# yangao07/abPOA

Hardware: NVIDIA H100
Metric: GCUPS (DP cells/s), global/convex 10 kbp (higher is better)
Workload: dtype int16 (packed int16x2 DPX arithmetic; int32 kernel only as overflow fallback)

## Files before the change

abpoa_b200/csrc/poa_chain.cu:

```cuda
#include <cuda_runtime.h>
#include <algorithm>
#include <atomic>
#include <chrono>
#include <mutex>
#include <thread>
#include <vector>
#include <stddef.h>
#include <stdio.h>
#include <stdlib.h>
#include <string.h>
#include <unistd.h>
#include "abpoa_gpu.h"
#include "poa_internal.h"
#include "poa_engine.h"
#include "poa_device.cuh"
#include "poa_chain.cuh"
#include "poa_chain_host.h"

#define CK(call) do { cudaError_t e_ = (call); if (e_ != cudaSuccess) \
    poa_die("libabpoa_b200/chain", "%s failed at %s:%d: %s", #call, __FILE__, __LINE__, cudaGetErrorString(e_)); } while (0)

extern "C" cudaError_t poa_launch_chain_dp_worker(int gap_mode, const int *gaps, PoaChainSlot *slots, PoaChainSync *sync, int n_groups,
                                                  const PoaChainParams *cp, int strand, int ps, int ext, const PoaParamsDev *prm, int ring_rows,
                                                  int ring_cells, cudaStream_t st);
extern "C" cudaError_t poa_launch_chain_align_p16(int gap_mode, const int *gaps, const PoaChainSlot *slots, const int32_t *idx, int n_jobs, int round,
                                                  const PoaChainParams *cp, int strand, int ps, int ext, const PoaParamsDev *prm, int ring_rows,
                                                  int ring_cells, cudaStream_t st);
extern "C" void poa_pick_ring(int gap_mode, int bits, int band_cells, size_t smem_budget, int *ring_rows, int *ring_cells);

static_assert(offsetof(PoaChainSync, q_tail) == 128 && offsetof(PoaChainSync, total) == 256 && offsetof(PoaChainSync, abort) == 384,
              "every polled / bumped word of PoaChainSync sits in its own 128-byte line");
static_assert(POA_GFA_HDR_WORDS == POA_GFA_HDR, "the device's GFA record header is the one poa_gfa_from_record reads");

template <bool PS, bool LG>
__global__ void __launch_bounds__(POA_CHAIN_T) poa_chain_seed_kernel(PoaChainSlot *slots, const PoaChainParams *cp, int n) {
    if ((int)blockIdx.x >= n) return;
    chain_seed<PS, LG>(&slots[blockIdx.x], cp);
}

template <bool PS, bool LG, bool KO = false>
__global__ void __launch_bounds__(POA_CHAIN_T) poa_chain_fuse_kernel(PoaChainSlot *slots, const int32_t *idx, const PoaChainParams *cp, int n, int round) {
    if ((int)blockIdx.x >= n) return;
    chain_fuse<PS, LG, KO>(&slots[idx[blockIdx.x]], cp, round);
}

__device__ __forceinline__ int sync_ld(const int32_t *p) { int v; asm volatile("ld.relaxed.gpu.global.s32 %0, [%1];" : "=r"(v) : "l"(p) : "memory"); return v; }
__device__ __forceinline__ void sync_st(int32_t *p, int v) { asm volatile("st.relaxed.gpu.global.s32 [%0], %1;" :: "l"(p), "r"(v) : "memory"); }
__device__ __forceinline__ unsigned long long sync_now_ns() { unsigned long long t; asm volatile("mov.u64 %0, %%globaltimer;" : "=l"(t)); return t; }

template <bool PS, bool LG, bool KO = false>
__global__ void __launch_bounds__(POA_CHAIN_T) poa_chain_fuse_worker_kernel(PoaChainSlot *slots, PoaChainSync *sync, const PoaChainParams *cp) {
    __shared__ int task_s;
    for (;;) {
        if (threadIdx.x < 32) {
            unsigned ticket = 0;
            if (threadIdx.x == 0) ticket = atomicAdd(&sync->q_head, 1u);
            ticket = __shfl_sync(0xffffffffu, ticket, 0);
            int g = -2; unsigned ns = 250, polls = 0;
            const unsigned long long t0 = sync_now_ns(), limit = sync->watchdog_ns;
            const int32_t *tasks = sync->tasks;
            for (;;) {
                if ((polls++ & 31u) == 0) {
                    const int tot = __shfl_sync(0xffffffffu, sync_ld(&sync->total), 0), ab = __shfl_sync(0xffffffffu, sync_ld(&sync->abort), 0);
                    if ((long long)ticket >= (long long)tot || ab) { g = -2; break; }
                    const unsigned late = __shfl_sync(0xffffffffu, (unsigned)(polls > 1 && sync_now_ns() - t0 > limit), 0);
                    if (late) { if (threadIdx.x == 0) sync_st(&sync->abort, 1); g = -2; break; }
                }
                g = __shfl_sync(0xffffffffu, sync_ld(&tasks[ticket]), 0);
                if (g >= 0) break;
                __nanosleep(ns); if (ns < 4000) ns <<= 1;
            }
            if (threadIdx.x == 0) task_s = g;
        }
        __syncthreads();
        const int g = task_s;
        __syncthreads();
        if (g < 0) return;
        __threadfence();
        PoaChainSlot *s = &slots[g];
        const unsigned long long t0 = sync_now_ns();
        chain_fuse<PS, LG, KO>(s, cp, 0);
        __syncthreads();
        __threadfence();
        __syncthreads();
// ... 746 lines not shown
            int khz = 0; if (cudaDeviceGetAttribute(&khz, cudaDevAttrClockRate, c.dev) != cudaSuccess || khz <= 0) khz = 1965000;
            for (int t = 0; t < nw; ++t) {
                dp_ms += (double)(fin[t].fwd_clk + fin[t].bt_clk) / (double)khz; fuse_ms += (double)fin[t].fuse_ns * 1e-6; wait_ms += (double)fin[t].wait_ns * 1e-6;
                n_marks += fin[t].fused > 0 ? fin[t].fused - 1 : 0;
            }
        } else {
            for (Cohort &k : coh)
                for (size_t j = 0; j + 2 < k.marks.size(); j += 3) {
                    float a = 0.f, b = 0.f;
                    CK(cudaEventElapsedTime(&a, k.marks[j], k.marks[j + 1])); CK(cudaEventElapsedTime(&b, k.marks[j + 1], k.marks[j + 2]));
                    dp_ms += a; fuse_ms += b; ++n_marks;
                }
        }
        if (PoaChainStats *stats = c.stats) {
            stats->device_ms += dev_ms; stats->cells += cells; stats->alignments += alns; stats->launches += launches;
            stats->h2d_bytes += h2d; stats->d2h_bytes += d2h; stats->groups_done += nw - n_failed; stats->groups_failed += n_failed;
            stats->fwd_clk += fwd_clk; stats->bt_clk += bt_clk;
            stats->dp_ms += dp_ms; stats->fuse_ms += fuse_ms; stats->dp_launches += n_marks; stats->fuse_launches += n_marks;
            stats->wait_ms += wait_ms; stats->free_running = c.free_run ? 1 : 0;
        }
        if (!c.verbose) return;
#ifdef POA_KPROF
        {
            double pf[6] = {0, 0, 0, 0, 0, 0}; double na = 0;
            for (int t = 0; t < nw; ++t) { for (int z = 0; z < 6; ++z) pf[z] += (double)fin[t].prof[z]; na += fin[t].fused > 0 ? fin[t].fused - 1 : 0; }
            double bd[5] = {0, 0, 0, 0, 0};
            for (int t = 0; t < nw; ++t) for (int z = 0; z < 5; ++z) bd[z] += (double)fin[t].btdiag[z];
            if (na > 0) fprintf(stderr, "[chain, backtrace per alignment] %.0f steps in %.0f speculative rounds, %.0f general steps costing %.0f k-cycles, "
                                        "%.1f rows with their F planes recomputed\n", bd[0] / na, bd[1] / na, bd[2] / na, bd[3] / na, bd[4] / na);
            if (na > 0) fprintf(stderr, "[chain, k-cycles/alignment] -DPOA_KPROF phases: setup %.0f pred %.0f compute %.0f store %.0f rowmax %.0f tail+prefetch %.0f\n",
                                pf[0] / na / 1e3, pf[1] / na / 1e3, pf[2] / na / 1e3, pf[3] / na / 1e3, pf[4] / na / 1e3, pf[5] / na / 1e3);
        }
#endif
        if (c.free_run)
            fprintf(stderr, "[chain] free-running: per group on average %.1f ms inside alignments + %.1f ms inside fuse (waited %.1f ms for fuse workers incl. the fuse itself), %lld alignments\n",
                    dp_ms / nw, fuse_ms / nw, wait_ms / nw, (long long)n_marks);
        else
            fprintf(stderr, "[chain] DP kernels %.1f ms + fuse kernels %.1f ms summed over %zu concurrent cohort streams (%lld rounds)\n", dp_ms, fuse_ms, coh.size(), (long long)n_marks);
        fprintf(stderr, "[chain] wave of %d groups (%zu cohorts, K=%d): stage %.0f + upload-enqueue %.0f + launch-enqueue %.0f ms, stage+launch+device %.0f ms (device %.1f ms), export copy %.0f ms, import+consensus %.0f ms; "
                        "static %.2f GB, pool %.2f GB, export %.1f MB; %d groups handed to the launch engine\n",
                nw, coh.size(), c.K, t_staged - t_wave0, t_uploaded - t_staged, t_enqueued - t_uploaded, t_dev_done - t_wave0, dev_ms, t_copied - t_dev_done, now_ms() - t_copied,
                (double)doff / 1e9, (double)pool_bytes / 1e9, (double)tot_words * 4 / 1e6, n_failed);
    }
};

}

int poa_chain_run(int dev, poa_arena *arena, abpoa_para_t *abpt, int n_workers, const abpoa_gpu_group_t *groups,
                  abpoa_gpu_group_result_t *results, const std::vector<int> &todo, int flags, std::vector<int> &fallback, PoaChainStats *stats,
                  struct PoaEmit *emit) {
    CK(cudaSetDevice(dev));
    const ChainCall c = chain_call(dev, arena, abpt, n_workers, groups, results, todo, flags, stats, emit);
    const std::vector<GroupPlan> plans = plan_groups(c, todo, fallback);
    if (plans.empty()) return 0;
    for (const std::pair<size_t, size_t> &w : split_waves(plans, poa_arena_capacity(arena), fallback))
        Wave(c, plans.data() + w.first, (int)(w.second - w.first), fallback).run();
    return 0;
}
```

abpoa_b200/csrc/poa_chain.cuh:

```cuda
#ifndef POA_CHAIN_CUH
#define POA_CHAIN_CUH

#include <math.h>
#include <stdint.h>
#include "poa_device.cuh"

#ifdef POA_CHAIN_EMUL
#define POA_DEV static inline
#define POA_PAR_FOR(i, n) for (int i = 0; i < (n); ++i)
#define POA_CTA_SYNC() do { } while (0)
#define POA_TID0 1
#define POA_SHARED static
#define POA_ATOMIC_OR(p, v) (*(p) |= (v))
#define POA_CTZ64(x) __builtin_ctzll(x)
#define POA_CHAIN_T 256
#else
#define POA_DEV __device__ __forceinline__
#define POA_PAR_FOR(i, n) for (int i = (int)threadIdx.x; i < (n); i += (int)blockDim.x)
#define POA_CTA_SYNC() __syncthreads()
#define POA_TID0 (threadIdx.x == 0)
#define POA_SHARED __shared__
#define POA_ATOMIC_OR(p, v) atomicOr((p), (v))
#define POA_CTZ64(x) (__ffsll((long long)(x)) - 1)
#define POA_CHAIN_T 256
#endif

#define POA_CF_NODE_CAP   0x01
#define POA_CF_EDGE_CAP   0x02
#define POA_CF_ALN_CAP    0x04
#define POA_CF_ORDER      0x08
#define POA_CF_BLOB_CAP   0x10
#define POA_CF_DP_STATUS  0x20
#define POA_CF_CIGAR      0x40
#define POA_CF_POOL       0x80

#define POA_ST_SKIP       9

typedef struct PoaChainParams {
    int32_t K, A;
    int32_t m, max_mat, min_mis, o1, e1, oe1, oe2;
    int32_t record;
    int32_t P;
    int32_t W;
    int32_t cons_algrm;
    int32_t amb_strand;
} PoaChainParams;

typedef struct PoaChainSlot {
    int32_t n_nodes, n_cap, pred_cap, blob_cap;
    int32_t failed;
    int32_t n_reads, fused;
    int32_t retry;
    int32_t cur;
    int64_t cells;
    int64_t fwd_clk, bt_clk;
    uint8_t *base;
    int32_t *in_cnt, *out_cnt, *aln_cnt, *n_read;
    int32_t *in_id, *in_w, *out_id, *out_w;
    int32_t *aln_id;
    int32_t *order[2];
    int32_t *node_row;
    int32_t *rem_row;
    int32_t *scr[6];
    const uint8_t *reads; const int32_t *read_off;
    const int32_t *read_w;
    PoaJobDesc jd;
    uint8_t *pool_base; unsigned long long *pool_cursor; uint64_t pool_units;
    int32_t turn;
    int32_t rsv0;
    unsigned long long wait_ns, fuse_ns;
    int64_t prof[6];
    int64_t btdiag[5];
    int32_t *rec_score, *rec_nops; uint64_t *rec_hash;
    uint64_t *read_set;
    uint8_t *read_rc;
    uint64_t *rc_cigar;
    PoaResultDev *rc_result;
    const uint8_t *read_qw;
} PoaChainSlot;

template <class Take>
static inline void chain_slot_layout(PoaChainSlot *s, int n_cap, int qmax, int n_reads, int K, int A, int m, int W, bool record, Take take,
                                     bool strand = false, bool ps = false) {
    const size_t nc = (size_t)n_cap, scr_n = nc > (size_t)qmax + 2 ? nc : (size_t)qmax + 2;
    s->n_cap = n_cap; s->pred_cap = (int32_t)(nc * 3); s->n_reads = n_reads;
    s->blob_cap = (int32_t)(256 + (nc + 1) * 8 + (size_t)s->pred_cap * 4 + 4 + (size_t)qmax + 64);
    if (ps) s->blob_cap += (int32_t)((size_t)s->pred_cap * 4 + 4 + 16);
    s->jd.cigar_cap = (int32_t)(qmax + n_cap + 8);
    s->base = (uint8_t *)take(nc);
    s->in_cnt = (int32_t *)take(nc * 4); s->out_cnt = (int32_t *)take(nc * 4); s->aln_cnt = (int32_t *)take(nc * 4); s->n_read = (int32_t *)take(nc * 4);
    s->in_id = (int32_t *)take(nc * K * 4); s->in_w = (int32_t *)take(nc * K * 4); s->out_id = (int32_t *)take(nc * K * 4); s->out_w = (int32_t *)take(nc * K * 4);
    s->aln_id = (int32_t *)take(nc * A * 4);
    s->order[0] = (int32_t *)take(nc * 4); s->order[1] = (int32_t *)take(nc * 4); s->node_row = (int32_t *)take(nc * 4); s->rem_row = (int32_t *)take(nc * 4);
    for (int k = 0; k < 6; ++k) s->scr[k] = (int32_t *)take(scr_n * 4);
    s->jd.blob = (uint8_t *)take((size_t)s->blob_cap);
    s->jd.rowinfo = (PoaRowInfo *)take(nc * sizeof(PoaRowInfo)); s->jd.rowoff = (PoaRowOff *)take(nc * sizeof(PoaRowOff));
    s->jd.cigar = (uint64_t *)take((size_t)s->jd.cigar_cap * 8);
    s->jd.qprof = (int16_t *)take((size_t)m * ((((size_t)qmax + 1 + 7) & ~(size_t)7) + 8) * 2);
    s->jd.result = (PoaResultDev *)take(sizeof(PoaResultDev));
    s->jd.btrec = (PoaBtRec *)take(nc * sizeof(PoaBtRec));
    if (record) { s->rec_score = (int32_t *)take((size_t)n_reads * 4); s->rec_nops = (int32_t *)take((size_t)n_reads * 4); s->rec_hash = (uint64_t *)take((size_t)n_reads * 8); }
    if (W > 0) s->read_set = (uint64_t *)take(nc * W * 8);
    if (strand) {
        s->read_rc = (uint8_t *)take((size_t)n_reads);
        s->rc_cigar = (uint64_t *)take((size_t)s->jd.cigar_cap * 8);
        s->rc_result = (PoaResultDev *)take(sizeof(PoaResultDev));
    }
}

template <class Take>
static inline void chain_slot_reads(PoaChainSlot *s, int n_reads, int64_t bases, Take take, bool qv = false) {
    s->reads = (const uint8_t *)take((size_t)bases);
    s->read_off = (const int32_t *)take(((size_t)n_reads + 1) * 4);
    s->read_w = (const int32_t *)take((size_t)n_reads * 4);
    if (qv) s->read_qw = (const uint8_t *)take((size_t)bases);
}

typedef struct PoaChainSync {
    unsigned int q_head; int32_t pad0[31];
    unsigned int q_tail; int32_t pad1[31];
    int32_t total; int32_t pad2[31];
    int32_t abort; int32_t pad3[31];
    unsigned long long watchdog_ns;
    int32_t *tasks;
} PoaChainSync;

#ifdef POA_CHAIN_EMUL
POA_DEV int cta_excl_scan(int32_t *a, int n) {
    int run = 0;
    for (int i = 0; i < n; ++i) { const int v = a[i]; a[i] = run; run += v; }
    return run;
}
POA_DEV void cta_incl_maxscan(int32_t *a, int n) {
    int run = INT32_MIN;
    for (int i = 0; i < n; ++i) { if (a[i] > run) run = a[i]; a[i] = run; }
}
#else
__device__ inline int cta_excl_scan(int32_t *a, int n) {
    __shared__ int warp_sum[32];
    __shared__ int carry_s;
    const int lane = threadIdx.x & 31, wid = threadIdx.x >> 5, nw = blockDim.x >> 5;
    if (threadIdx.x == 0) carry_s = 0;
    __syncthreads();
    for (int base = 0; base < n; base += blockDim.x) {
        const int i = base + threadIdx.x;
        const int v = i < n ? a[i] : 0;
        int x = v;
#pragma unroll
        for (int d = 1; d < 32; d <<= 1) { const int t = __shfl_up_sync(0xffffffffu, x, d); if (lane >= d) x += t; }
        if (lane == 31) warp_sum[wid] = x;
        __syncthreads();
        if (wid == 0) {
            int s = lane < nw ? warp_sum[lane] : 0;
#pragma unroll
            for (int d = 1; d < 32; d <<= 1) { const int t = __shfl_up_sync(0xffffffffu, s, d); if (lane >= d) s += t; }
            warp_sum[lane] = s;
        }
        __syncthreads();
        const int carry = carry_s;
        const int before = carry + (wid > 0 ? warp_sum[wid - 1] : 0) + x - v;
        if (i < n) a[i] = before;
        __syncthreads();
        if (threadIdx.x == 0) carry_s = carry + warp_sum[nw - 1];
        __syncthreads();
    }
    return carry_s;
}
__device__ inline void cta_incl_maxscan(int32_t *a, int n) {
    __shared__ int warp_max[32];
    __shared__ int carry_m;
    const int lane = threadIdx.x & 31, wid = threadIdx.x >> 5, nw = blockDim.x >> 5;
    if (threadIdx.x == 0) carry_m = INT32_MIN;
    __syncthreads();
    for (int base = 0; base < n; base += blockDim.x) {
        const int i = base + threadIdx.x;
        int x = i < n ? a[i] : INT32_MIN;
#pragma unroll
        for (int d = 1; d < 32; d <<= 1) { const int t = __shfl_up_sync(0xffffffffu, x, d); if (lane >= d) x = max(x, t); }
        if (lane == 31) warp_max[wid] = x;
        __syncthreads();
        if (wid == 0) {
            int s = lane < nw ? warp_max[lane] : INT32_MIN;
#pragma unroll
            for (int d = 1; d < 32; d <<= 1) { const int t = __shfl_up_sync(0xffffffffu, s, d); if (lane >= d) s = max(s, t); }
            warp_max[lane] = s;
        }
        __syncthreads();
        int r = max(carry_m, x);
        if (wid > 0) r = max(r, warp_max[wid - 1]);
        if (i < n) a[i] = r;
        __syncthreads();
        if (threadIdx.x == 0) carry_m = max(carry_m, warp_max[nw - 1]);
        __syncthreads();
    }
}
#endif

POA_DEV void chain_exchange_order(int32_t *ids, int32_t *ws, int n) {
    for (int j = 0; j + 1 < n; ++j)
        for (int k = j + 1; k < n; ++k)
            if (ws[j] < ws[k]) { int32_t t = ids[j]; ids[j] = ids[k]; ids[k] = t; t = ws[j]; ws[j] = ws[k]; ws[k] = t; }
}

POA_DEV int chain_group_last_row(const PoaChainSlot *s, int A, const int32_t *order, int old_n, int v) {
    int r = s->node_row[v];
    const int na = s->aln_cnt[v];
    if (na == 0) return r;
    const int32_t *al = s->aln_id + (size_t)v * A;
    for (; r + 1 < old_n; ++r) {
        const int u = order[r + 1];
        int member = 0;
        for (int a = 0; a < na; ++a) if (al[a] == u) { member = 1; break; }
        if (!member) break;
    }
    return r;
}

POA_DEV int chain_ref_pn(const PoaChainParams *cp, int qlen, int n_rows) {
    const int len = qlen > n_rows ? qlen : n_rows;
    const int a = qlen * cp->max_mat, b = len * cp->e1 + cp->o1;
    const int max_score = a > b ? a : b;
    return max_score <= 32767 - cp->min_mis - cp->oe1 - cp->oe2 ? 16 : 8;
}

#define POA_LG_ROW_CELLS(pn) (2 * ((pn) - 1))

POA_DEV size_t chain_al16(size_t x) { return (x + 15) & ~(size_t)15; }

POA_DEV bool chain_weak_hit(int best_score, int qlen, int node_n, int max_mat) {
    const int lim = qlen < node_n - 2 ? qlen : node_n - 2;
    return best_score < lim * max_mat * .3333;
}

#define POA_PS_MAX_NODE_W (1 << 20)
POA_DEV int chain_path_score(int edge_w, int node_w) {
    if (node_w == 0 || edge_w == 0) return 0;
    const int s = (int)round(log((double)edge_w / (double)node_w));
    return s > -20 ? s : -20;
}

POA_DEV uint8_t chain_comp(uint8_t b) { return b < 4 ? (uint8_t)(3 - b) : (uint8_t)4; }

typedef struct ChainRead { const uint8_t *q, *w; int len; bool rc; } ChainRead;

POA_DEV ChainRead chain_read(const PoaChainSlot *s, int r) {
    ChainRead rd;
    rd.q = s->reads + s->read_off[r]; rd.w = s->read_qw ? s->read_qw + s->read_off[r] : NULL;
    rd.len = s->read_off[r + 1] - s->read_off[r]; rd.rc = s->read_rc && (s->read_rc[r] & 1);
    return rd;
}

POA_DEV uint8_t chain_read_base(const ChainRead &rd, int qi) { return rd.rc ? chain_comp(rd.q[rd.len - 1 - qi]) : rd.q[qi]; }

POA_DEV int chain_read_weight(const ChainRead &rd, int qi) { return !rd.w ? 1 : rd.w[rd.rc ? rd.len - 1 - qi : qi]; }

POA_DEV void chain_set_remain(PoaChainSlot *s, int K, const int32_t *order, int n) {
    POA_SHARED int t_ptr[POA_CHAIN_T], t_val[POA_CHAIN_T], t_np[POA_CHAIN_T], t_nv[POA_CHAIN_T];
    int32_t *rem = s->rem_row;
    if (POA_TID0) rem[n - 1] = -1;
    POA_CTA_SYNC();
    for (int hi = n - 1; hi > 0; hi -= POA_CHAIN_T) {
        const int lo = hi - POA_CHAIN_T > 0 ? hi - POA_CHAIN_T : 0;
        const int cnt = hi - lo;
        POA_PAR_FOR(l, POA_CHAIN_T) {
            if (l < cnt) {
                const int v = order[lo + l];
                const int sr = s->node_row[s->out_id[(size_t)v * K]];
                if (sr >= hi) { t_ptr[l] = -1; t_val[l] = rem[sr] + 1; }
                else { t_ptr[l] = sr - lo; t_val[l] = 1; }
            } else { t_ptr[l] = -1; t_val[l] = 0; }
        }
        POA_CTA_SYNC();
        for (int step = 1; step < POA_CHAIN_T; step <<= 1) {
            POA_PAR_FOR(l, POA_CHAIN_T) {
                const int p = t_ptr[l];
                if (p >= 0) { t_nv[l] = t_val[l] + t_val[p]; t_np[l] = t_ptr[p]; } else { t_nv[l] = t_val[l]; t_np[l] = -1; }
            }
            POA_CTA_SYNC();
            POA_PAR_FOR(l, POA_CHAIN_T) { t_val[l] = t_nv[l]; t_ptr[l] = t_np[l]; }
            POA_CTA_SYNC();
        }
        POA_PAR_FOR(l, POA_CHAIN_T) { if (l < cnt) rem[lo + l] = t_val[l]; }
        POA_CTA_SYNC();
    }
}

#define CHAIN_KAHN_LINK 0xff
POA_DEV void chain_kahn_order(PoaChainSlot *s, const PoaChainParams *cp, int32_t *order, int n) {
    const int K = cp->K, A = cp->A;
    uint8_t *deg = reinterpret_cast<uint8_t *>(s->scr[2]);
    int32_t *nx = s->scr[3];
    POA_PAR_FOR(v, n) {
        const int ni = s->in_cnt[v];
        deg[v] = (ni == 1 && s->aln_cnt[v] == 0) ? (uint8_t)CHAIN_KAHN_LINK : (uint8_t)ni;
    }
    POA_CTA_SYNC();
    POA_PAR_FOR(u, n) {
        int x = -1;
        if (s->out_cnt[u] == 1) { const int v = s->out_id[(size_t)u * K]; if (deg[v] == CHAIN_KAHN_LINK) x = v; }
        nx[u] = x;
    }
    POA_CTA_SYNC();
    if (POA_TID0) {
        int head = 0, tail = 1, last = 0, done = 0;
        order[0] = 0;
        while (head < tail) {
            const int cur = head + 1 == tail ? last : order[head];
            s->node_row[cur] = head++;
            if (cur == 1) { done = head == n; break; }
            const int x = nx[cur];
            if (x >= 0) {
                if (tail >= n) break;
                order[tail++] = last = x;
                continue;
            }
            const int ne = s->out_cnt[cur];
            const int32_t *oid = s->out_id + (size_t)cur * K;
            int full = 0;
            for (int e = 0; e < ne && !full; ++e) {
                const int v = oid[e];
                int d = deg[v];
                if (d != CHAIN_KAHN_LINK) {
                    deg[v] = (uint8_t)--d;
                    if (d != 0) continue;
                    const int na = s->aln_cnt[v];
                    const int32_t *al = s->aln_id + (size_t)v * A;
                    int ready = 1;
                    for (int a = 0; a < na; ++a) if (deg[al[a]] != 0) { ready = 0; break; }
                    if (!ready) continue;
                    if (tail + 1 + na > n) { full = 1; break; }
                    order[tail++] = last = v;
                    for (int a = 0; a < na; ++a) order[tail++] = last = al[a];
                } else {
                    if (tail >= n) { full = 1; break; }
                    order[tail++] = last = v;
                }
            }
            if (full) break;
        }
        if (!done) POA_ATOMIC_OR(&s->failed, POA_CF_ORDER);
    }
    POA_CTA_SYNC();
}

template <bool PS = false, bool LG = false>
POA_DEV void chain_flatten(PoaChainSlot *s, const PoaChainParams *cp, const int32_t *order, int n, int r, int pool_parity, int generous) {
    const int K = cp->K;
    int32_t *cnt = s->scr[0];
    POA_PAR_FOR(i, n) cnt[i] = i == 0 ? 0 : s->in_cnt[order[i]];
    POA_CTA_SYNC();
    const int n_pred = cta_excl_scan(cnt, n);
    POA_CTA_SYNC();
    const int qlen = s->read_off[r + 1] - s->read_off[r];
    uint8_t *blob = const_cast<uint8_t *>(s->jd.blob);
    PoaJobHeader *h = reinterpret_cast<PoaJobHeader *>(blob);
    size_t off = chain_al16(sizeof(PoaJobHeader));
    const size_t off_rowmeta = off; off += chain_al16(((size_t)n + 1) * 8);
    const size_t off_pred = off; off += chain_al16((size_t)n_pred * 4 + 4);
    const size_t off_ps = off; if (PS) off += chain_al16((size_t)n_pred * 4 + 4);
    const size_t off_qs = off; off += chain_al16((size_t)qlen + 1) + 16;
    if (off > (size_t)s->blob_cap || n_pred > s->pred_cap) {
        if (POA_TID0) { POA_ATOMIC_OR(&s->failed, POA_CF_BLOB_CAP); h->n_rows = 0; }
        POA_CTA_SYNC();
        return;
    }
    int32_t *rowmeta = reinterpret_cast<int32_t *>(blob + off_rowmeta), *pred = reinterpret_cast<int32_t *>(blob + off_pred);
    int32_t *pscore = reinterpret_cast<int32_t *>(blob + off_ps);
    uint8_t *qs = blob + off_qs;
    POA_PAR_FOR(i, n) {
        const int v = order[i];
        const int po = cnt[i];
        rowmeta[2 * i] = po;
        rowmeta[2 * i + 1] = (int32_t)((uint32_t)s->rem_row[i] << 8) | s->base[v];
        if (i > 0) {
            const int ni = s->in_cnt[v];
            const int32_t *iid = s->in_id + (size_t)v * K;
            for (int e = 0; e < ni; ++e) {
                const int pr = s->node_row[iid[e]];
                if (pr >= i) POA_ATOMIC_OR(&s->failed, POA_CF_ORDER);
                pred[po + e] = pr;
                if (PS) {
                    const int u = iid[e], no = s->out_cnt[u];
                    const int32_t *ow = s->out_w + (size_t)u * K;
                    int node_w = 0;
                    for (int o = 0; o < no; ++o) node_w += ow[o];
                    pscore[po + e] = chain_path_score(s->in_w[(size_t)v * K + e], node_w);
                }
            }
        }
    }
    const uint8_t *q = s->reads + s->read_off[r];
    const int qpad = (int)(off - off_qs);
    POA_PAR_FOR(j, qpad) qs[j] = (j >= 1 && j <= qlen) ? q[j - 1] : (uint8_t)0;
    if (POA_TID0) {
        rowmeta[2 * n] = n_pred; rowmeta[2 * n + 1] = 0;
        h->qlen = qlen; h->w = s->read_w[r]; h->node_n = n;
        h->off_rowmeta = (int32_t)off_rowmeta; h->off_pred = (int32_t)off_pred; h->off_predscore = PS ? (int32_t)off_ps : -1; h->off_live = -1;
        h->off_qs = (int32_t)off_qs; h->rsv[0] = h->rsv[1] = h->rsv[2] = h->rsv[3] = 0;
        h->blob_bytes = (int32_t)off; h->pn = chain_ref_pn(cp, qlen, n); h->pad[0] = h->pad[1] = 0;
#ifndef POA_CHAIN_EMUL
        if (s->pool_base) {
            const int w = s->read_w[r];
            const int drift = qlen > s->rem_row[0] ? qlen - s->rem_row[0] : s->rem_row[0] - qlen;
            unsigned long long per_row = (unsigned long long)((2 * w + 1 + drift + 64 + (LG ? POA_LG_ROW_CELLS(h->pn) : 0) + 7) / 8 + 2);
            const unsigned long long full = (unsigned long long)((qlen + 1 + 7) / 8 + 1);
            if (generous || per_row > full) per_row = full;
            const unsigned long long units = per_row * (unsigned long long)cp->P * (unsigned long long)n;
            if (!s->pool_cursor) {
                s->jd.planes = s->pool_base; s->jd.plane_cap_units = s->pool_units;
            } else {
                const unsigned long long at = atomicAdd(&s->pool_cursor[pool_parity & 1], units);
                if (at + units > s->pool_units) POA_ATOMIC_OR(&s->failed, POA_CF_POOL);
                else { s->jd.planes = s->pool_base + (size_t)at * (POA_GROUP * 2); s->jd.plane_cap_units = units; }
            }
        }
#endif
    }
    POA_CTA_SYNC();
    if (POA_TID0) h->n_rows = s->failed ? 0 : n;
    POA_CTA_SYNC();
}

template <bool PS = false, bool LG = false>
POA_DEV void chain_seed(PoaChainSlot *s, const PoaChainParams *cp) {
    const int K = cp->K;
    ChainRead rd = chain_read(s, 0);
    rd.rc = false;
    const int len = rd.len;
    const uint8_t *q = rd.q;
    const int n = len + 2;
    if (n > s->n_cap || len < 1) {
        if (POA_TID0) { POA_ATOMIC_OR(&s->failed, POA_CF_NODE_CAP); reinterpret_cast<PoaJobHeader *>(const_cast<uint8_t *>(s->jd.blob))->n_rows = 0; }
        POA_CTA_SYNC();
        return;
    }
    int32_t *order = s->order[0];
    POA_PAR_FOR(v, n) {
        s->aln_cnt[v] = 0;
        if (v == 0) { s->base[v] = 0; s->in_cnt[v] = 0; s->out_cnt[v] = 1; s->out_id[0] = 2; s->out_w[0] = chain_read_weight(rd, 0); s->n_read[v] = 1; order[0] = 0; s->node_row[0] = 0; }
        else if (v == 1) {
            s->base[v] = 0; s->out_cnt[v] = 0; s->in_cnt[v] = 1; s->in_id[(size_t)K] = len + 1; s->in_w[(size_t)K] = chain_read_weight(rd, len - 1); s->n_read[v] = 0;
            order[n - 1] = 1; s->node_row[1] = n - 1;
        } else {
            const int i = v - 2;
            s->base[v] = q[i];
            s->in_cnt[v] = 1; s->in_id[(size_t)v * K] = i == 0 ? 0 : v - 1; s->in_w[(size_t)v * K] = chain_read_weight(rd, i);
            s->out_cnt[v] = 1; s->out_id[(size_t)v * K] = i == len - 1 ? 1 : v + 1; s->out_w[(size_t)v * K] = chain_read_weight(rd, i == len - 1 ? i : i + 1);
            s->n_read[v] = 1;
            order[i + 1] = v; s->node_row[v] = i + 1;
        }
    }
    if (cp->W > 0) {
        const int W = cp->W;
        POA_PAR_FOR(v, n) { uint64_t *rs = s->read_set + (size_t)v * W; for (int wd = 0; wd < W; ++wd) rs[wd] = (wd == 0 && v != 1) ? 1ull : 0ull; }
    }
    if (POA_TID0) { s->n_nodes = n; s->cur = 0; s->fused = 1; s->retry = 0; if (s->read_rc) s->read_rc[0] = 0; }
    POA_CTA_SYNC();
    chain_set_remain(s, K, order, n);
    if (s->n_reads > 1) chain_flatten<PS, LG>(s, cp, order, n, 1, 1, 0);
}

#define CK_OLD  0
#define CK_NEWM 1
#define CK_NEWI 2

template <bool PS = false, bool LG = false, bool KO = false>
POA_DEV void chain_fuse(PoaChainSlot *s, const PoaChainParams *cp, int round) {
    const int K = cp->K, A = cp->A;
    const int r = s->fused;
    PoaJobHeader *hdr = reinterpret_cast<PoaJobHeader *>(const_cast<uint8_t *>(s->jd.blob));
    if (s->failed || r >= s->n_reads) return;
    const PoaResultDev *res = s->jd.result;
    if (res->status == POA_ST_SKIP) return;
    if (res->status == POA_ST_PLANE_OVF && !s->retry && s->pool_cursor) {
        POA_CTA_SYNC();
        if (POA_TID0) s->retry = 1;
        chain_flatten<PS, LG>(s, cp, s->order[s->cur], s->n_nodes, r, round + 1, 1);
        return;
    }
    if (res->status != POA_ST_OK) {
        if (POA_TID0) { POA_ATOMIC_OR(&s->failed, POA_CF_DP_STATUS); hdr->n_rows = 0; }
        POA_CTA_SYNC();
        return;
    }
    const ChainRead rd = chain_read(s, r);
    const int qlen = rd.len;
    const uint64_t *ops = s->jd.cigar;
    const int n_ops = res->n_ops;
    const int old_n = s->n_nodes;
    const int32_t *order = s->order[s->cur];
    int32_t *order_new = s->order[s->cur ^ 1];
    int32_t *item_row = s->scr[0], *tgt = s->scr[1], *isnew = s->scr[2], *kind_anchor = s->scr[3], *defidx = s->scr[4], *new_anchor = s->scr[5];

    if (POA_TID0) {
        s->cells += res->cells; s->fwd_clk += res->fwd_clk; s->bt_clk += res->bt_clk;
#ifdef POA_KPROF
        for (int z = 0; z < 6; ++z) s->prof[z] += res->prof[z];
        for (int z = 0; z < 5; ++z) s->btdiag[z] += res->btdiag[z];
#endif
        if (cp->record) {
            s->rec_score[r] = res->best_score; s->rec_nops[r] = n_ops;
            uint64_t hsh = 1469598103934665603ull;
            for (int t = n_ops - 1; t >= 0; --t) {
                uint64_t w = ops[t];
                if ((w & 0xf) != 1) w = ((uint64_t)(uint32_t)order[w >> 34] << 34) | (w & 0x3ffffffffull);
                for (int b = 0; b < 8; ++b) { hsh ^= (w >> (8 * b)) & 0xff; hsh *= 1099511628211ull; }
            }
            s->rec_hash[r] = hsh;
        }
    }

    POA_PAR_FOR(qi, qlen + 1) { item_row[qi] = -2; }
    POA_CTA_SYNC();
    POA_PAR_FOR(t, n_ops) {
        const uint64_t w = ops[t];
        const int op = (int)(w & 0xf);
        if (op == 0) {
            const int qp = (int)((w >> 4) & 0x3fffffff), row = (int)(w >> 34);
            if (qp < qlen && row > 0 && row < old_n - 1) item_row[qp] = row; else POA_ATOMIC_OR(&s->failed, POA_CF_CIGAR);
        } else if (op == 1) {
            const int qp = (int)(w >> 34), len = (int)((w >> 4) & 0x3fffffff);
            if (qp < qlen && qp - len + 1 >= 0) { for (int k = 0; k < len; ++k) item_row[qp - k] = -1; } else POA_ATOMIC_OR(&s->failed, POA_CF_CIGAR);
        }
    }
    POA_CTA_SYNC();

    POA_PAR_FOR(qi, qlen) {
        const int row = item_row[qi];
        int kind = CK_NEWI, target = -1, anchor = -1;
        if (row == -2) POA_ATOMIC_OR(&s->failed, POA_CF_CIGAR);
        if (row >= 0) {
            const int v = order[row];
            const uint8_t b = chain_read_base(rd, qi);
            if (s->base[v] == b) { kind = CK_OLD; target = v; }
            else {
                const int na = s->aln_cnt[v]; const int32_t *al = s->aln_id + (size_t)v * A;
                for (int a = 0; a < na; ++a) if (s->base[al[a]] == b) { target = al[a]; break; }
                if (target >= 0) kind = CK_OLD;
                else { kind = CK_NEWM; anchor = KO ? -1 : chain_group_last_row(s, A, order, old_n, v); target = v; }
            }
        }
        tgt[qi] = target; isnew[qi] = kind != CK_OLD;
        kind_anchor[qi] = (kind << 28) | (anchor & 0x0fffffff);
    }
    POA_CTA_SYNC();
    if (s->failed) { if (POA_TID0) hdr->n_rows = 0; POA_CTA_SYNC(); return; }

    int32_t *newidx = defidx;
    POA_PAR_FOR(qi, qlen) newidx[qi] = isnew[qi];
    POA_CTA_SYNC();
    const int n_new = cta_excl_scan(newidx, qlen);
    POA_CTA_SYNC();
    const int n = old_n + n_new;
    if (n > s->n_cap) { if (POA_TID0) { POA_ATOMIC_OR(&s->failed, POA_CF_NODE_CAP); hdr->n_rows = 0; } POA_CTA_SYNC(); return; }

    if (!KO) {
    POA_PAR_FOR(qi, qlen) {
        const int kind = kind_anchor[qi] >> 28;
        int anchor = -1;
        if (kind == CK_NEWM) anchor = kind_anchor[qi] & 0x0fffffff;
        else if (kind == CK_NEWI && !(qi > 0 && isnew[qi - 1])) anchor = chain_group_last_row(s, A, order, old_n, qi == 0 ? 0 : tgt[qi - 1]);
        new_anchor[qi] = anchor;
    }
    POA_CTA_SYNC();
    {
        int32_t *d = item_row;
        POA_PAR_FOR(qi, qlen) d[qi] = new_anchor[qi] >= 0 ? qi : -1;
        POA_CTA_SYNC();
        cta_incl_maxscan(d, qlen);
        POA_CTA_SYNC();
        POA_PAR_FOR(qi, qlen) {
            if (isnew[qi]) {
                const int a = d[qi] >= 0 ? new_anchor[d[qi]] : -1;
                if (a < 0) POA_ATOMIC_OR(&s->failed, POA_CF_ORDER);
                kind_anchor[qi] = (kind_anchor[qi] & (int32_t)0xf0000000) | (a & 0x0fffffff);
            }
        }
        POA_CTA_SYNC();
    }
    }

    POA_PAR_FOR(qi, qlen) {
        if (isnew[qi]) {
            const int id = old_n + newidx[qi];
            const int col = tgt[qi];
            s->base[id] = chain_read_base(rd, qi); s->in_cnt[id] = 0; s->out_cnt[id] = 0; s->aln_cnt[id] = 0; s->n_read[id] = 0;
            if (cp->W > 0) for (int wd = 0; wd < cp->W; ++wd) s->read_set[(size_t)id * cp->W + wd] = 0;
            new_anchor[newidx[qi]] = kind_anchor[qi] & 0x0fffffff;
            item_row[qi] = col;
            tgt[qi] = id;
        }
    }
    POA_CTA_SYNC();

    POA_PAR_FOR(qi, qlen + 1) {
        const int from = qi == 0 ? 0 : tgt[qi - 1], to = qi < qlen ? tgt[qi] : 1;
        const int from_new = qi > 0 && isnew[qi - 1], to_new = qi < qlen && isnew[qi];
        const int w = chain_read_weight(rd, qi < qlen ? qi : qlen - 1);
        int32_t *iid = s->in_id + (size_t)to * K, *iw = s->in_w + (size_t)to * K;
        int32_t *oid = s->out_id + (size_t)from * K, *ow = s->out_w + (size_t)from * K;
        int nin = s->in_cnt[to], nout = s->out_cnt[from];
        int found = 0;
        if (!from_new && !to_new) {
            for (int i = 0; i < nin; ++i)
                if (iid[i] == from) { iw[i] += w; found = 1; if (i > 0 && iw[i - 1] < iw[i]) chain_exchange_order(iid, iw, nin); break; }
            if (found)
                for (int i = 0; i < nout; ++i)
                    if (oid[i] == to) { ow[i] += w; if (!KO && i > 0 && ow[i - 1] < ow[i]) chain_exchange_order(oid, ow, nout); break; }
        }
        if (!found) {
            if (nin >= K || nout >= K) POA_ATOMIC_OR(&s->failed, POA_CF_EDGE_CAP);
            else {
                iid[nin] = from; iw[nin] = w; s->in_cnt[to] = ++nin;
                if (nin > 1 && iw[nin - 2] < w) chain_exchange_order(iid, iw, nin);
                oid[nout] = to; ow[nout] = w; s->out_cnt[from] = ++nout;
                if (!KO && nout > 1 && ow[nout - 2] < w) chain_exchange_order(oid, ow, nout);
            }
        }
        s->n_read[from] += 1;
        if (cp->W > 0) s->read_set[(size_t)from * cp->W + (r >> 6)] |= 1ull << (r & 63);
    }
    POA_CTA_SYNC();

    POA_PAR_FOR(qi, qlen) {
        if ((kind_anchor[qi] >> 28) == CK_NEWM) {
            const int col = item_row[qi], id = tgt[qi];
            const int na = s->aln_cnt[col];
            if (na + 1 > A) POA_ATOMIC_OR(&s->failed, POA_CF_ALN_CAP);
            else {
                int32_t *mine = s->aln_id + (size_t)id * A; int nm = 0;
                for (int a = 0; a < na; ++a) {
                    const int sib = s->aln_id[(size_t)col * A + a];
                    s->aln_id[(size_t)sib * A + s->aln_cnt[sib]] = id; s->aln_cnt[sib] += 1;
                    mine[nm++] = sib;
                }
                s->aln_id[(size_t)col * A + na] = id; s->aln_cnt[col] = na + 1;
                mine[nm++] = col; s->aln_cnt[id] = nm;
            }
        }
    }
    POA_CTA_SYNC();
    if (s->failed) { if (POA_TID0) hdr->n_rows = 0; POA_CTA_SYNC(); return; }

    if (KO) {
        chain_kahn_order(s, cp, order_new, n);
        POA_PAR_FOR(v, n) { const int no = s->out_cnt[v]; if (no > 1) chain_exchange_order(s->out_id + (size_t)v * K, s->out_w + (size_t)v * K, no); }
        POA_CTA_SYNC();
        if (s->failed) { if (POA_TID0) hdr->n_rows = 0; POA_CTA_SYNC(); return; }
    } else {
    POA_PAR_FOR(k, n_new) { if (k > 0 && new_anchor[k] < new_anchor[k - 1]) POA_ATOMIC_OR(&s->failed, POA_CF_ORDER); }
    POA_CTA_SYNC();
    if (s->failed) { if (POA_TID0) hdr->n_rows = 0; POA_CTA_SYNC(); return; }
    POA_PAR_FOR(i, old_n) {
        int lo = 0, hi = n_new;
        while (lo < hi) { const int mid = (lo + hi) >> 1; if (new_anchor[mid] < i) lo = mid + 1; else hi = mid; }
        const int v = order[i], nr = i + lo;
        order_new[nr] = v; s->node_row[v] = nr;
    }
    POA_PAR_FOR(k, n_new) {
        const int nr = new_anchor[k] + 1 + k, v = old_n + k;
        order_new[nr] = v; s->node_row[v] = nr;
    }
    POA_CTA_SYNC();
    }
    if (POA_TID0) { s->n_nodes = n; s->cur ^= 1; s->fused = r + 1; s->retry = 0; }
    POA_CTA_SYNC();

    chain_set_remain(s, K, order_new, n);
    if (r + 1 < s->n_reads) chain_flatten<PS, LG>(s, cp, order_new, n, r + 1, round + 1, 0);
    else if (POA_TID0) hdr->n_rows = 0;
    POA_CTA_SYNC();
}

POA_DEV void chain_consensus(PoaChainSlot *s, const PoaChainParams *cp, int32_t *out, int out_cap) {
    if (!POA_TID0) return;
    const int K = cp->K, n = s->n_nodes;
    const int32_t *order = s->order[s->cur];
    int32_t *score = s->scr[0], *nxt = s->scr[1];
    if (s->failed || n < 3) { out[0] = -1; return; }
    for (int r = n - 1; r >= 0; --r) {
        const int v = order[r];
        const int ne = s->out_cnt[v];
        const int32_t *oid = s->out_id + (size_t)v * K, *ow = s->out_w + (size_t)v * K;
        if (v == 1) { score[v] = 0; nxt[v] = -1; }
        else if (v == 0) {
            int pick = -1, pick_score = -1, pick_w = -1;
            for (int e = 0; e < ne; ++e) {
                const int u = oid[e], w = ow[e];
                if (w > pick_w || (w == pick_w && score[u] > pick_score)) { pick = u; pick_score = score[u]; pick_w = w; }
            }
            nxt[v] = pick;
        } else {
            int pick = -1, pick_w = INT32_MIN;
            for (int e = 0; e < ne; ++e) {
                const int u = oid[e], w = ow[e];
                if (pick_w < w) { pick_w = w; pick = u; }
                else if (pick_w == w && score[pick] <= score[u]) pick = u;
            }
            score[v] = pick_w + score[pick];
// ... 213 lines not shown
```

Baseline: 126.6.

## Speed up chain fuse: segmented scans, gathered remain, prefetches, merge-walk splice

```diff
diff --git a/abpoa_b200/csrc/poa_chain.cu b/abpoa_b200/csrc/poa_chain.cu
--- a/abpoa_b200/csrc/poa_chain.cu
+++ b/abpoa_b200/csrc/poa_chain.cu
@@ -49,7 +49,7 @@
 __device__ __forceinline__ unsigned long long sync_now_ns() { unsigned long long t; asm volatile("mov.u64 %0, %%globaltimer;" : "=l"(t)); return t; }
 
 template <bool PS, bool LG, bool KO = false>
-__global__ void __launch_bounds__(POA_CHAIN_T) poa_chain_fuse_worker_kernel(PoaChainSlot *slots, PoaChainSync *sync, const PoaChainParams *cp) {
+__global__ void __launch_bounds__(POA_CHAIN_T, PS ? 3 : 4) poa_chain_fuse_worker_kernel(PoaChainSlot *slots, PoaChainSync *sync, const PoaChainParams *cp) {
     __shared__ int task_s;
     for (;;) {
         if (threadIdx.x < 32) {
@@ -862,9 +862,19 @@
                                 pf[0] / na / 1e3, pf[1] / na / 1e3, pf[2] / na / 1e3, pf[3] / na / 1e3, pf[4] / na / 1e3, pf[5] / na / 1e3);
         }
 #endif
+        char fphase[256] = "";
+#ifdef POA_KPROF
+        {
+            double fp[8] = {0, 0, 0, 0, 0, 0, 0, 0};
+            for (int t = 0; t < nw; ++t) for (int z = 0; z < 8; ++z) fp[z] += (double)fin[t].fprof[z];
+            const double d = n_marks > 0 ? (double)n_marks * 1e3 : 1.0;
+            snprintf(fphase, sizeof fphase, "; -DPOA_KPROF us/fuse: steps 1-2 %.0f, new ids %.0f, anchors %.0f, steps 5-7 %.0f, splice %.0f, remain %.0f, "
+                                            "flatten gather+scan %.0f, flatten fill %.0f", fp[0] / d, fp[1] / d, fp[2] / d, fp[3] / d, fp[4] / d, fp[5] / d, fp[6] / d, fp[7] / d);
+        }
+#endif
         if (c.free_run)
-            fprintf(stderr, "[chain] free-running: per group on average %.1f ms inside alignments + %.1f ms inside fuse (waited %.1f ms for fuse workers incl. the fuse itself), %lld alignments\n",
-                    dp_ms / nw, fuse_ms / nw, wait_ms / nw, (long long)n_marks);
+            fprintf(stderr, "[chain] free-running: per group on average %.1f ms inside alignments + %.1f ms inside fuse (waited %.1f ms for fuse workers incl. the fuse itself), %lld alignments%s\n",
+                    dp_ms / nw, fuse_ms / nw, wait_ms / nw, (long long)n_marks, fphase);
         else
             fprintf(stderr, "[chain] DP kernels %.1f ms + fuse kernels %.1f ms summed over %zu concurrent cohort streams (%lld rounds)\n", dp_ms, fuse_ms, coh.size(), (long long)n_marks);
         fprintf(stderr, "[chain] wave of %d groups (%zu cohorts, K=%d): stage %.0f + upload-enqueue %.0f + launch-enqueue %.0f ms, stage+launch+device %.0f ms (device %.1f ms), export copy %.0f ms, import+consensus %.0f ms; "
diff --git a/abpoa_b200/csrc/poa_chain.cuh b/abpoa_b200/csrc/poa_chain.cuh
--- a/abpoa_b200/csrc/poa_chain.cuh
+++ b/abpoa_b200/csrc/poa_chain.cuh
@@ -14,6 +14,7 @@
 #define POA_ATOMIC_OR(p, v) (*(p) |= (v))
 #define POA_CTZ64(x) __builtin_ctzll(x)
 #define POA_CHAIN_T 256
+#define POA_PREFETCH(p) ((void)(p))
 #else
 #define POA_DEV __device__ __forceinline__
 #define POA_PAR_FOR(i, n) for (int i = (int)threadIdx.x; i < (n); i += (int)blockDim.x)
@@ -23,6 +24,7 @@
 #define POA_ATOMIC_OR(p, v) atomicOr((p), (v))
 #define POA_CTZ64(x) (__ffsll((long long)(x)) - 1)
 #define POA_CHAIN_T 256
+#define POA_PREFETCH(p) asm volatile("prefetch.global.L2 [%0];" :: "l"(p))
 #endif
 
 #define POA_CF_NODE_CAP   0x01
@@ -77,6 +79,9 @@
     uint64_t *rc_cigar;
     PoaResultDev *rc_result;
     const uint8_t *read_qw;
+#ifdef POA_KPROF
+    unsigned long long fprof[8], fprof_t;
+#endif
 } PoaChainSlot;
 
 template <class Take>
@@ -126,74 +131,68 @@
 } PoaChainSync;
 
 #ifdef POA_CHAIN_EMUL
-POA_DEV int cta_excl_scan(int32_t *a, int n) {
-    int run = 0;
-    for (int i = 0; i < n; ++i) { const int v = a[i]; a[i] = run; run += v; }
+template <bool MAX, class Ld>
+POA_DEV int cta_scan(int32_t *a, int n, Ld ld) {
+    int run = MAX ? INT32_MIN : 0;
+    for (int i = 0; i < n; ++i) {
+        const int v = ld(i);
+        if (MAX) { if (v > run) run = v; a[i] = run; } else { a[i] = run; run += v; }
+    }
     return run;
 }
-POA_DEV void cta_incl_maxscan(int32_t *a, int n) {
-    int run = INT32_MIN;
-    for (int i = 0; i < n; ++i) { if (a[i] > run) run = a[i]; a[i] = run; }
-}
 #else
-__device__ inline int cta_excl_scan(int32_t *a, int n) {
-    __shared__ int warp_sum[32];
-    __shared__ int carry_s;
+template <bool MAX, class Ld>
+__device__ inline int cta_scan(int32_t *a, int n, Ld ld) {
+    __shared__ int seg_tot[32];
+    constexpr int ID = MAX ? INT32_MIN : 0;
     const int lane = threadIdx.x & 31, wid = threadIdx.x >> 5, nw = blockDim.x >> 5;
-    if (threadIdx.x == 0) carry_s = 0;
+    const int S = ((n + nw - 1) / nw + 31) & ~31;
+    const int lo = min(n, wid * S), hi = min(n, lo + S);
+    int run = ID;
+    for (int b = lo; b < hi; b += 128) {
+        int v[4];
+#pragma unroll
+        for (int u = 0; u < 4; ++u) { const int i = b + 32 * u + lane; v[u] = i < hi ? ld(i) : ID; }
+#pragma unroll
+        for (int u = 0; u < 4; ++u) {
+            int x = v[u];
+#pragma unroll
+            for (int d = 1; d < 32; d <<= 1) { const int t = __shfl_up_sync(0xffffffffu, x, d); if (lane >= d) x = MAX ? max(x, t) : x + t; }
+            const int i = b + 32 * u + lane;
+            if (i < hi) a[i] = MAX ? max(run, x) : run + x - v[u];
+            const int seg = __shfl_sync(0xffffffffu, x, 31);
+            run = MAX ? max(run, seg) : run + seg;
+        }
+    }
+    if (lane == 0) seg_tot[wid] = run;
     __syncthreads();
-    for (int base = 0; base < n; base += blockDim.x) {
-        const int i = base + threadIdx.x;
-        const int v = i < n ? a[i] : 0;
-        int x = v;
+    int off = ID, tot = ID;
+    for (int w = 0; w < nw; ++w) {
+        const int t = seg_tot[w];
+        if (w < wid) off = MAX ? max(off, t) : off + t;
+        tot = MAX ? max(tot, t) : tot + t;
+    }
+    if (off != ID)
+        for (int b = lo; b < hi; b += 128) {
 #pragma unroll
-        for (int d = 1; d < 32; d <<= 1) { const int t = __shfl_up_sync(0xffffffffu, x, d); if (lane >= d) x += t; }
-        if (lane == 31) warp_sum[wid] = x;
-        __syncthreads();
-        if (wid == 0) {
-            int s = lane < nw ? warp_sum[lane] : 0;
-#pragma unroll
-            for (int d = 1; d < 32; d <<= 1) { const int t = __shfl_up_sync(0xffffffffu, s, d); if (lane >= d) s += t; }
-            warp_sum[lane] = s;
-        }
-        __syncthreads();
-        const int carry = carry_s;
-        const int before = carry + (wid > 0 ? warp_sum[wid - 1] : 0) + x - v;
-        if (i < n) a[i] = before;
-        __syncthreads();
-        if (threadIdx.x == 0) carry_s = carry + warp_sum[nw - 1];
-        __syncthreads();
-    }
-    return carry_s;
-}
-__device__ inline void cta_incl_maxscan(int32_t *a, int n) {
-    __shared__ int warp_max[32];
-    __shared__ int carry_m;
-    const int lane = threadIdx.x & 31, wid = threadIdx.x >> 5, nw = blockDim.x >> 5;
-    if (threadIdx.x == 0) carry_m = INT32_MIN;
+            for (int u = 0; u < 4; ++u) { const int i = b + 32 * u + lane; if (i < hi) a[i] = MAX ? max(a[i], off) : a[i] + off; }
+        }
     __syncthreads();
-    for (int base = 0; base < n; base += blockDim.x) {
-        const int i = base + threadIdx.x;
-        int x = i < n ? a[i] : INT32_MIN;
-#pragma unroll
-        for (int d = 1; d < 32; d <<= 1) { const int t = __shfl_up_sync(0xffffffffu, x, d); if (lane >= d) x = max(x, t); }
-        if (lane == 31) warp_max[wid] = x;
-        __syncthreads();
-        if (wid == 0) {
-            int s = lane < nw ? warp_max[lane] : INT32_MIN;
-#pragma unroll
-            for (int d = 1; d < 32; d <<= 1) { const int t = __shfl_up_sync(0xffffffffu, s, d); if (lane >= d) s = max(s, t); }
-            warp_max[lane] = s;
-        }
-        __syncthreads();
-        int r = max(carry_m, x);
-        if (wid > 0) r = max(r, warp_max[wid - 1]);
-        if (i < n) a[i] = r;
-        __syncthreads();
-        if (threadIdx.x == 0) carry_m = max(carry_m, warp_max[nw - 1]);
-        __syncthreads();
-    }
-}
+    return tot;
+}
+#endif
+POA_DEV int cta_excl_scan(int32_t *a, int n) { return cta_scan<false>(a, n, [a](int i) { return a[i]; }); }
+POA_DEV void cta_incl_maxscan(int32_t *a, int n) { cta_scan<true>(a, n, [a](int i) { return a[i]; }); }
+
+#if defined(POA_KPROF) && !defined(POA_CHAIN_EMUL)
+__device__ __forceinline__ void chain_prof_lap(PoaChainSlot *s, int z) {
+    if (threadIdx.x != 0) return;
+    unsigned long long t; asm volatile("mov.u64 %0, %%globaltimer;" : "=l"(t));
+    if (z >= 0) s->fprof[z] += t - s->fprof_t;
+    s->fprof_t = t;
+}
+#else
+#define chain_prof_lap(s, z) do { } while (0)
 #endif
 
 POA_DEV void chain_exchange_order(int32_t *ids, int32_t *ws, int n) {
@@ -254,35 +253,44 @@
 
 POA_DEV int chain_read_weight(const ChainRead &rd, int qi) { return !rd.w ? 1 : rd.w[rd.rc ? rd.len - 1 - qi : qi]; }
 
+#define POA_REM_T (2 * POA_CHAIN_T)
+#define POA_GATHER_B 4
 POA_DEV void chain_set_remain(PoaChainSlot *s, int K, const int32_t *order, int n) {
-    POA_SHARED int t_ptr[POA_CHAIN_T], t_val[POA_CHAIN_T], t_np[POA_CHAIN_T], t_nv[POA_CHAIN_T];
-    int32_t *rem = s->rem_row;
+    POA_SHARED int32_t t_pd[2][POA_REM_T];
+    int32_t *rem = s->rem_row, *nx = s->scr[5];
+    const int32_t *out_id = s->out_id, *node_row = s->node_row;
+    for (int i0 = 0; i0 < n - 1; i0 += POA_GATHER_B * POA_CHAIN_T) {
+        POA_PAR_FOR(t, POA_CHAIN_T) {
+            int x[POA_GATHER_B];
+#pragma unroll
+            for (int u = 0; u < POA_GATHER_B; ++u) { const int i = i0 + u * POA_CHAIN_T + t; if (i < n - 1) x[u] = order[i]; }
+#pragma unroll
+            for (int u = 0; u < POA_GATHER_B; ++u) { const int i = i0 + u * POA_CHAIN_T + t; if (i < n - 1) x[u] = out_id[(size_t)x[u] * K]; }
+#pragma unroll
+            for (int u = 0; u < POA_GATHER_B; ++u) { const int i = i0 + u * POA_CHAIN_T + t; if (i < n - 1) nx[i] = node_row[x[u]]; }
+        }
+    }
     if (POA_TID0) rem[n - 1] = -1;
     POA_CTA_SYNC();
-    for (int hi = n - 1; hi > 0; hi -= POA_CHAIN_T) {
-        const int lo = hi - POA_CHAIN_T > 0 ? hi - POA_CHAIN_T : 0;
+    for (int hi = n - 1; hi > 0; hi -= POA_REM_T) {
+        const int lo = hi - POA_REM_T > 0 ? hi - POA_REM_T : 0;
         const int cnt = hi - lo;
-        POA_PAR_FOR(l, POA_CHAIN_T) {
-            if (l < cnt) {
-                const int v = order[lo + l];
-                const int sr = s->node_row[s->out_id[(size_t)v * K]];
-                if (sr >= hi) { t_ptr[l] = -1; t_val[l] = rem[sr] + 1; }
-                else { t_ptr[l] = sr - lo; t_val[l] = 1; }
-            } else { t_ptr[l] = -1; t_val[l] = 0; }
+        POA_PAR_FOR(l, cnt) {
+            const int sr = nx[lo + l];
+            if (sr >= lo && sr < hi) t_pd[0][l] = 1 << 16 | (sr - lo);
+            else { t_pd[0][l] = l; rem[lo + l] = sr >= hi ? rem[sr] + 1 : 1; }
         }
         POA_CTA_SYNC();
-        for (int step = 1; step < POA_CHAIN_T; step <<= 1) {
-            POA_PAR_FOR(l, POA_CHAIN_T) {
-                const int p = t_ptr[l];
-                if (p >= 0) { t_nv[l] = t_val[l] + t_val[p]; t_np[l] = t_ptr[p]; } else { t_nv[l] = t_val[l]; t_np[l] = -1; }
-            }
+        int c = 0;
+        for (int span = 1; span < cnt; span <<= 1) {
+            POA_PAR_FOR(l, cnt) { const int e = t_pd[c][l]; t_pd[c ^ 1][l] = (e & ~0xffff) + t_pd[c][e & 0xffff]; }
             POA_CTA_SYNC();
-            POA_PAR_FOR(l, POA_CHAIN_T) { t_val[l] = t_nv[l]; t_ptr[l] = t_np[l]; }
-            POA_CTA_SYNC();
-        }
-        POA_PAR_FOR(l, POA_CHAIN_T) { if (l < cnt) rem[lo + l] = t_val[l]; }
+            c ^= 1;
+        }
+        POA_PAR_FOR(l, cnt) { const int e = t_pd[c][l], root = e & 0xffff; if (root != l) rem[lo + l] = (e >> 16) + rem[lo + root]; }
         POA_CTA_SYNC();
     }
+    chain_prof_lap(s, 5);
 }
 
 #define CHAIN_KAHN_LINK 0xff
@@ -347,10 +355,9 @@
 POA_DEV void chain_flatten(PoaChainSlot *s, const PoaChainParams *cp, const int32_t *order, int n, int r, int pool_parity, int generous) {
     const int K = cp->K;
     int32_t *cnt = s->scr[0];
-    POA_PAR_FOR(i, n) cnt[i] = i == 0 ? 0 : s->in_cnt[order[i]];
-    POA_CTA_SYNC();
-    const int n_pred = cta_excl_scan(cnt, n);
-    POA_CTA_SYNC();
+    const int32_t *in_cnt = s->in_cnt;
+    const int n_pred = cta_scan<false>(cnt, n, [=](int i) { return i == 0 ? 0 : in_cnt[order[i]]; });
+    chain_prof_lap(s, 6);
     const int qlen = s->read_off[r + 1] - s->read_off[r];
     uint8_t *blob = const_cast<uint8_t *>(s->jd.blob);
     PoaJobHeader *h = reinterpret_cast<PoaJobHeader *>(blob);
@@ -367,16 +374,21 @@
     int32_t *rowmeta = reinterpret_cast<int32_t *>(blob + off_rowmeta), *pred = reinterpret_cast<int32_t *>(blob + off_pred);
     int32_t *pscore = reinterpret_cast<int32_t *>(blob + off_ps);
     uint8_t *qs = blob + off_qs;
+    const int32_t *in_id = s->in_id, *node_row = s->node_row;
     POA_PAR_FOR(i, n) {
+        if (i + POA_CHAIN_T < n) {
+            const int nv = order[i + POA_CHAIN_T];
+            POA_PREFETCH(s->base + nv); POA_PREFETCH(in_id + (size_t)nv * K);
+        }
         const int v = order[i];
         const int po = cnt[i];
         rowmeta[2 * i] = po;
         rowmeta[2 * i + 1] = (int32_t)((uint32_t)s->rem_row[i] << 8) | s->base[v];
         if (i > 0) {
-            const int ni = s->in_cnt[v];
-            const int32_t *iid = s->in_id + (size_t)v * K;
+            const int ni = in_cnt[v];
+            const int32_t *iid = in_id + (size_t)v * K;
             for (int e = 0; e < ni; ++e) {
-                const int pr = s->node_row[iid[e]];
+                const int pr = node_row[iid[e]];
                 if (pr >= i) POA_ATOMIC_OR(&s->failed, POA_CF_ORDER);
                 pred[po + e] = pr;
                 if (PS) {
@@ -419,6 +431,7 @@
     POA_CTA_SYNC();
     if (POA_TID0) h->n_rows = s->failed ? 0 : n;
     POA_CTA_SYNC();
+    chain_prof_lap(s, 7);
 }
 
 template <bool PS = false, bool LG = false>
@@ -456,6 +469,7 @@
     }
     if (POA_TID0) { s->n_nodes = n; s->cur = 0; s->fused = 1; s->retry = 0; if (s->read_rc) s->read_rc[0] = 0; }
     POA_CTA_SYNC();
+    chain_prof_lap(s, -1);
     chain_set_remain(s, K, order, n);
     if (s->n_reads > 1) chain_flatten<PS, LG>(s, cp, order, n, 1, 1, 0);
 }
@@ -475,6 +489,7 @@
     if (res->status == POA_ST_PLANE_OVF && !s->retry && s->pool_cursor) {
         POA_CTA_SYNC();
         if (POA_TID0) s->retry = 1;
+        chain_prof_lap(s, -1);
         chain_flatten<PS, LG>(s, cp, s->order[s->cur], s->n_nodes, r, round + 1, 1);
         return;
     }
@@ -491,6 +506,7 @@
     const int32_t *order = s->order[s->cur];
     int32_t *order_new = s->order[s->cur ^ 1];
     int32_t *item_row = s->scr[0], *tgt = s->scr[1], *isnew = s->scr[2], *kind_anchor = s->scr[3], *defidx = s->scr[4], *new_anchor = s->scr[5];
+    chain_prof_lap(s, -1);
 
     if (POA_TID0) {
         s->cells += res->cells; s->fwd_clk += res->fwd_clk; s->bt_clk += res->bt_clk;
@@ -517,7 +533,7 @@
         const int op = (int)(w & 0xf);
         if (op == 0) {
             const int qp = (int)((w >> 4) & 0x3fffffff), row = (int)(w >> 34);
-            if (qp < qlen && row > 0 && row < old_n - 1) item_row[qp] = row; else POA_ATOMIC_OR(&s->failed, POA_CF_CIGAR);
+            if (qp < qlen && row > 0 && row < old_n - 1) { item_row[qp] = row; POA_PREFETCH(order + row); } else POA_ATOMIC_OR(&s->failed, POA_CF_CIGAR);
         } else if (op == 1) {
             const int qp = (int)(w >> 34), len = (int)((w >> 4) & 0x3fffffff);
             if (qp < qlen && qp - len + 1 >= 0) { for (int k = 0; k < len; ++k) item_row[qp - k] = -1; } else POA_ATOMIC_OR(&s->failed, POA_CF_CIGAR);
@@ -526,6 +542,10 @@
     POA_CTA_SYNC();
 
     POA_PAR_FOR(qi, qlen) {
+        if (qi + POA_CHAIN_T < qlen) {
+            const int nr = item_row[qi + POA_CHAIN_T];
+            if (nr >= 0) { const int nv = order[nr]; POA_PREFETCH(s->base + nv); POA_PREFETCH(s->aln_cnt + nv); }
+        }
         const int row = item_row[qi];
         int kind = CK_NEWI, target = -1, anchor = -1;
         if (row == -2) POA_ATOMIC_OR(&s->failed, POA_CF_CIGAR);
@@ -544,6 +564,7 @@
         kind_anchor[qi] = (kind << 28) | (anchor & 0x0fffffff);
     }
     POA_CTA_SYNC();
+    chain_prof_lap(s, 0);
     if (s->failed) { if (POA_TID0) hdr->n_rows = 0; POA_CTA_SYNC(); return; }
 
     int32_t *newidx = defidx;
@@ -551,6 +572,7 @@
     POA_CTA_SYNC();
     const int n_new = cta_excl_scan(newidx, qlen);
     POA_CTA_SYNC();
+    chain_prof_lap(s, 1);
     const int n = old_n + n_new;
     if (n > s->n_cap) { if (POA_TID0) { POA_ATOMIC_OR(&s->failed, POA_CF_NODE_CAP); hdr->n_rows = 0; } POA_CTA_SYNC(); return; }
 
@@ -579,6 +601,7 @@
         POA_CTA_SYNC();
     }
     }
+    chain_prof_lap(s, 2);
 
     POA_PAR_FOR(qi, qlen) {
         if (isnew[qi]) {
@@ -594,6 +617,12 @@
     POA_CTA_SYNC();
 
     POA_PAR_FOR(qi, qlen + 1) {
+        if (qi + POA_CHAIN_T <= qlen) {
+            const int nq = qi + POA_CHAIN_T, nf = tgt[nq - 1], nt = nq < qlen ? tgt[nq] : 1;
+            POA_PREFETCH(s->in_cnt + nt); POA_PREFETCH(s->in_id + (size_t)nt * K); POA_PREFETCH(s->in_w + (size_t)nt * K);
+            POA_PREFETCH(s->out_cnt + nf); POA_PREFETCH(s->out_id + (size_t)nf * K); POA_PREFETCH(s->out_w + (size_t)nf * K);
+            POA_PREFETCH(s->n_read + nf);
+        }
         const int from = qi == 0 ? 0 : tgt[qi - 1], to = qi < qlen ? tgt[qi] : 1;
         const int from_new = qi > 0 && isnew[qi - 1], to_new = qi < qlen && isnew[qi];
         const int w = chain_read_weight(rd, qi < qlen ? qi : qlen - 1);
@@ -640,6 +669,7 @@
         }
     }
     POA_CTA_SYNC();
+    chain_prof_lap(s, 3);
     if (s->failed) { if (POA_TID0) hdr->n_rows = 0; POA_CTA_SYNC(); return; }
 
     if (KO) {
@@ -651,11 +681,16 @@
     POA_PAR_FOR(k, n_new) { if (k > 0 && new_anchor[k] < new_anchor[k - 1]) POA_ATOMIC_OR(&s->failed, POA_CF_ORDER); }
     POA_CTA_SYNC();
     if (s->failed) { if (POA_TID0) hdr->n_rows = 0; POA_CTA_SYNC(); return; }
-    POA_PAR_FOR(i, old_n) {
+    POA_PAR_FOR(t, POA_CHAIN_T) {
+        const int per = (old_n + POA_CHAIN_T - 1) / POA_CHAIN_T, i0 = t * per, i1 = i0 + per < old_n ? i0 + per : old_n;
         int lo = 0, hi = n_new;
-        while (lo < hi) { const int mid = (lo + hi) >> 1; if (new_anchor[mid] < i) lo = mid + 1; else hi = mid; }
-        const int v = order[i], nr = i + lo;
-        order_new[nr] = v; s->node_row[v] = nr;
+        while (lo < hi) { const int mid = (lo + hi) >> 1; if (new_anchor[mid] < i0) lo = mid + 1; else hi = mid; }
+        int a = lo < n_new ? new_anchor[lo] : INT32_MAX;
+        for (int i = i0; i < i1; ++i) {
+            while (a < i) { ++lo; a = lo < n_new ? new_anchor[lo] : INT32_MAX; }
+            const int v = order[i], nr = i + lo;
+            order_new[nr] = v; s->node_row[v] = nr;
+        }
     }
     POA_PAR_FOR(k, n_new) {
         const int nr = new_anchor[k] + 1 + k, v = old_n + k;
@@ -665,6 +700,7 @@
     }
     if (POA_TID0) { s->n_nodes = n; s->cur ^= 1; s->fused = r + 1; s->retry = 0; }
     POA_CTA_SYNC();
+    chain_prof_lap(s, 4);
 
     chain_set_remain(s, K, order_new, n);
     if (r + 1 < s->n_reads) chain_flatten<PS, LG>(s, cp, order_new, n, r + 1, round + 1, 0);
```

After: 127.0, median of 6. No clear change (+0.4%).
